# zm0612/funny_lidar_slam

Hardware: AMD Instinct MI355X
Metric: scans/sec (64-ring×1800 pts → 1e6-pt iVox map), SE(3) err vs CPU ref (higher is better)
Workload: dtype f64; 1 GPU; BASELINE configs[1]: Velodyne-64 synthetic scan (64x1800 = 115,200 pts), point-to-plane (LoamPointToPlaneIVOX semantics, YAML config_nclt.yaml) into a 1e6-pt iVox map, 1 scan per GPU per step (the same scan on every GPU); scan_points=115200, map_points=1000000, converged=True, pre_warm_matches=256

## Files before the change

### funny_lidar_slam_amd/_lib.py

```python
from __future__ import annotations

import ctypes as C
import os
import subprocess

_HERE = os.path.dirname(os.path.abspath(__file__))
LIB_PATH = os.environ.get("FLS_REG_LIB") or os.path.join(_HERE, "libfls_reg.so")
CSRC_DIR = os.path.join(_HERE, "csrc")

EXPORTED_SYMBOLS = [
    "fls_create", "fls_destroy", "fls_add_cloud_to_local_map", "fls_match", "fls_get_fitness_score",
    "fls_scan_upload", "fls_scan_upload_raw", "fls_match_resident", "fls_match_batch", "fls_map_export", "fls_map_import", "fls_map_image_bytes", "fls_map_image_export", "fls_map_image_import", "fls_get_iteration_log", "fls_get_correspondences", "fls_map_size",
    "fls_set_profiling", "fls_get_kernel_time", "fls_get_traffic_counters", "fls_get_debug_stamps", "fls_debug_fullpiv_qr6", "fls_debug_ldlt6", "fls_debug_voxel_grid", "fls_debug_voxel_grid_timed", "fls_debug_exact_sort", "fls_debug_exact_sort_marks", "fls_voxel_grid_cloud", "fls_loop_match", "fls_status_string", "fls_abi_version", "fls_abi_revision",
    "fls_device_count",
    "fls_replicas_create", "fls_replicas_refresh", "fls_replicas_match_batch", "fls_replicas_import_ms", "fls_replicas_destroy",
    "fls_features_create", "fls_features_destroy", "fls_features_project", "fls_features_extract", "fls_features_get", "fls_features_get_time",
]
HANDOFF_SYMBOLS = ["fls_preprocess_scan_device", "fls_scan_attach_preprocessed", "fls_preprocess_get_host_bytes"]
PREPROCESS_SYMBOLS = [
    "fls_preprocess_create", "fls_preprocess_destroy", "fls_preprocess_scan", "fls_preprocess_get", "fls_preprocess_get_time",
    "fls_features_project_deskew",
] + HANDOFF_SYMBOLS

FLS_OK, FLS_NOT_CONVERGED, FLS_SKIPPED = 0, 1, 2
FLS_ERR_INVALID, FLS_ERR_DEVICE, FLS_ERR_RANGE, FLS_ERR_NOMEM, FLS_ERR_STATE = -1, -2, -3, -4, -5

ICP_OPTIMIZED, P2PLANE_IVOX, INCREMENTAL_NDT, LOAM_FULL, P2PLANE_KDTREE = range(5)

# ... 172 lines not shown
                                     C.c_void_p]
        L.fls_voxel_grid_cloud.restype = C.c_int
        L.fls_voxel_grid_cloud.argtypes = [C.c_int, C.c_int, C.POINTER(C.c_float), C.c_size_t, C.c_int, C.c_float, C.POINTER(C.c_float), C.c_size_t,
                                           C.POINTER(C.c_size_t)]
        L.fls_debug_voxel_grid.restype = C.c_int
        L.fls_debug_voxel_grid.argtypes = [C.c_int, C.POINTER(C.c_float), C.c_size_t, C.c_int, C.c_float, C.POINTER(C.c_float), C.c_size_t,
                                           C.POINTER(C.c_size_t)]
        L.fls_debug_voxel_grid_timed.restype = C.c_int
        L.fls_debug_voxel_grid_timed.argtypes = [C.c_int, C.POINTER(C.c_float), C.c_size_t, C.c_int, C.c_float, C.c_int, C.POINTER(C.c_double), C.POINTER(C.c_size_t)]
        L.fls_debug_exact_sort.restype = C.c_int
        L.fls_debug_exact_sort.argtypes = [C.c_int, C.POINTER(C.c_uint32), C.POINTER(C.c_uint32), C.c_size_t, C.c_int]
        L.fls_debug_fullpiv_qr6.restype = C.c_int
        L.fls_debug_fullpiv_qr6.argtypes = [C.c_int, C.POINTER(C.c_double), C.POINTER(C.c_double), C.c_int, C.POINTER(C.c_double)]
        L.fls_debug_ldlt6.restype = C.c_int
        L.fls_debug_ldlt6.argtypes = [C.c_int, C.POINTER(C.c_double), C.POINTER(C.c_double), C.c_int, C.POINTER(C.c_double), C.POINTER(C.c_int32)]
        L.fls_get_debug_stamps.restype = C.c_int
        L.fls_get_debug_stamps.argtypes = [hp, C.POINTER(C.c_int64)]
        L.fls_features_create.restype = C.c_int
        L.fls_features_create.argtypes = [C.POINTER(FeatureParams), C.c_int, C.POINTER(hp)]
        L.fls_features_destroy.restype = None
        L.fls_features_destroy.argtypes = [hp]
        L.fls_features_project.restype = C.c_int
        L.fls_features_project.argtypes = [hp, C.c_void_p, C.c_size_t, C.POINTER(PointLayout), C.POINTER(C.c_size_t)]
        L.fls_features_extract.restype = C.c_int
        L.fls_features_extract.argtypes = [hp, C.POINTER(C.c_size_t), C.POINTER(C.c_size_t)]
        L.fls_features_get.restype = C.c_size_t
        L.fls_features_get.argtypes = [hp, C.c_int, C.c_void_p, C.c_size_t]
        L.fls_features_get_time.restype = C.c_int
        L.fls_features_get_time.argtypes = [hp, dp, dp]
        u64p = C.POINTER(C.c_uint64)
# ... 35 lines not shown
```

### funny_lidar_slam_amd/csrc/device_common.hpp

```cpp
#pragma once
#include <hip/hip_runtime.h>
#include <stdint.h>

namespace fls {

constexpr int kMaxIter = 64;
constexpr int kPartialStride = 32;
constexpr unsigned long long kEmptyKey = ~0ull;
constexpr int kKeyLimit = (1 << 20) - 2;

struct HashEntry {
    unsigned long long key;
    unsigned begin;
    unsigned count;
};
static_assert(sizeof(HashEntry) == 16, "one dwordx4 per probe");

struct DevGrid {
    const HashEntry* table;
    const float4* pts;
    unsigned mask;
    unsigned n_pts;
};

// ... 162 lines not shown
}
__host__ __device__ __forceinline__ void unpack_key(unsigned long long k, int& x, int& y, int& z) {
    x = (int)((unsigned)(k >> 42) << 11) >> 11;
    y = (int)((unsigned)((k >> 21) & 0x1FFFFFu) << 11) >> 11;
    z = (int)((unsigned)(k & 0x1FFFFFu) << 11) >> 11;
}
__host__ __device__ __forceinline__ unsigned hash_key(unsigned long long k) {
    k ^= k >> 33;
    k *= 0xff51afd7ed558ccdULL;
    k ^= k >> 33;
    k *= 0xc4ceb9fe1a85ec53ULL;
    k ^= k >> 33;
    return (unsigned)k;
}

__device__ __forceinline__ unsigned evict_merged_rank(const unsigned* __restrict__ crank, const unsigned C, const unsigned* S, const unsigned nS, const unsigned k) {
    unsigned j = 0;
    while (j < nS && j <= k && S[j] < (k - j < C ? crank[k - j] : 0xFFFFFFFFu)) ++j;
    unsigned v = 0u;
    if (j <= k && k - j < C) v = crank[k - j];
    if (j > 0u && S[j - 1] > v) v = S[j - 1];
    return v;
}

}
```

### funny_lidar_slam_amd/csrc/fls_reg.hip

```cpp
#include <chrono>
#include "matcher_p2plane_ivox.hpp"
#include "matchers_kd.hpp"
#include "matcher_ndt.hpp"
#include "features_host.hpp"
#include "preprocess_host.hpp"
#include "loop_closure.hpp"
#include "replicas.hpp"
#include <new>

using namespace fls;

namespace {

int gfx950_device_count() {
    int n = 0;
    if (hipGetDeviceCount(&n) != hipSuccess) return 0;
    int ok = 0;
    for (int d = 0; d < n; ++d) {
        hipDeviceProp_t prop;
        if (hipGetDeviceProperties(&prop, d) != hipSuccess) continue;
        if (std::strncmp(prop.gcnArchName, "gfx950", 6) == 0) ++ok;
    }
    return ok;
}
// ... 263 lines not shown
    if (launches) *launches = h->prof_launches;
    if (point_iters) *point_iters = h->prof_point_iters;
    h->prof_ms = 0.0;
    h->prof_launches = 0;
    h->prof_point_iters = 0;
    return FLS_OK;
}

fls_status fls_get_debug_stamps(fls_handle h, int64_t out[16]) {
    if (!h || !out || !h->h_state.p) return FLS_ERR_INVALID;
    (void)guarded([&]() -> fls_status { FLS_HIP(hipSetDevice(h->device)); h->refresh_log(); return FLS_OK; });
    for (int i = 0; i < 16; ++i) out[i] = h->h_state.p->dbg[i];
    return FLS_OK;
}

fls_status fls_debug_fullpiv_qr6(int device_id, const double* H, const double* g, int n, double* x) {
    if (!H || !g || !x || n < 0) return FLS_ERR_INVALID;
    if (n == 0) return FLS_OK;
    return guarded([&]() -> fls_status {
        FLS_HIP(hipSetDevice(device_id));
        DevBuf<double> dH, dg, dx;
        dH.reserve(size_t(n) * 36); dg.reserve(size_t(n) * 6); dx.reserve(size_t(n) * 6);
        FLS_HIP(hipMemcpy(dH.p, H, size_t(n) * 36 * sizeof(double), hipMemcpyHostToDevice));
        FLS_HIP(hipMemcpy(dg.p, g, size_t(n) * 6 * sizeof(double), hipMemcpyHostToDevice));
        hipLaunchKernelGGL(debug_fullpiv_qr6_kernel, dim3(unsigned(n)), dim3(64), 0, nullptr, (const double*)dH.p, (const double*)dg.p, n, dx.p);
        FLS_HIP(hipGetLastError());
        FLS_HIP(hipMemcpy(x, dx.p, size_t(n) * 6 * sizeof(double), hipMemcpyDeviceToHost));
        return FLS_OK;
    });
}
// ... 303 lines not shown
```

### funny_lidar_slam_amd/csrc/kernels_ivox_coop.hpp

```cpp
#pragma once
#include "kernels_p2plane.hpp"

namespace fls {

__device__ __forceinline__ void nearby18(const int k, int& dx, int& dy, int& dz) {
    constexpr unsigned long long DX = 0x1548889561ull, DY = 0x895429495ull, DZ = 0x282956155ull;
    dx = (int)((DX >> (2 * k)) & 3ull) - 1;
    dy = (int)((DY >> (2 * k)) & 3ull) - 1;
    dz = (int)((DZ >> (2 * k)) & 3ull) - 1;
}

template <int STEP>
__device__ __forceinline__ unsigned dpp_pair_u32(const unsigned v) {
    static_assert(STEP >= 0 && STEP <= 3, "");
    if (STEP == 0) return (unsigned)__builtin_amdgcn_update_dpp(0, (int)v, 0xB1, 0xf, 0xf, true);
    if (STEP == 1) return (unsigned)__builtin_amdgcn_update_dpp(0, (int)v, 0x4E, 0xf, 0xf, true);
    if (STEP == 2) return (unsigned)__builtin_amdgcn_update_dpp(0, (int)v, 0x141, 0xf, 0xf, true);
    return (unsigned)__builtin_amdgcn_update_dpp(0, (int)v, 0x140, 0xf, 0xf, true);
}
template <int G>
__device__ __forceinline__ unsigned long long group_min_u64(unsigned long long v) {
#define FLS_MIN_STEP(S)                                                                               \
    {                                                                                                 \
        const unsigned lo = dpp_pair_u32<S>((unsigned)(v & 0xffffffffull));                          \
// ... 64 lines not shown
#undef FLS_DMIN_STEP
    return v;
}

template <int R>
__device__ __forceinline__ unsigned slot_select(const unsigned idx, const unsigned p1, const unsigned p2, const unsigned p3, const unsigned p4,
                                                const unsigned o0, const unsigned o1, const unsigned o2, const unsigned o3, const unsigned o4) {
    unsigned sel = R == 5 ? o4 : R == 4 ? o3 : R == 3 ? o2 : R == 2 ? o1 : o0;
    if (R > 4) sel = idx < p4 ? o3 : sel;
    if (R > 3) sel = idx < p3 ? o2 : sel;
    if (R > 2) sel = idx < p2 ? o1 : sel;
    if (R > 1) sel = idx < p1 ? o0 : sel;
    return idx + sel;
}

template <int G, bool COUNT, bool DENSE, bool FIRST, bool BAL = false>
__global__ void __launch_bounds__(256)
ivox_knn_kernel(const float* __restrict__ sx, const float* __restrict__ sy, const float* __restrict__ sz, const int n,
                const GnState* __restrict__ st, const Pose16 T0, const DevGrid grid, const BrickDir bd,
                const float inv_res, float4* __restrict__ nn_pts , unsigned char* __restrict__ nn_cnt,
                unsigned char* __restrict__ flag, TrafficCounters* __restrict__ tc, const int chunk,
                unsigned* __restrict__ nn_ids ,
                const int nn_prev ,
                float* __restrict__ dev_copy ) {
    static_assert(G == 4 || G == 8, "group size");
    constexpr int QPB = 256 / G;
    constexpr int R = (19 + G - 1) / G;
    const int nb = (n + QPB - 1) / QPB;
    const int xcd = blockIdx.x & 7, seq = blockIdx.x >> 3;
    const int lb = ((seq / chunk) * 8 + xcd) * chunk + (seq % chunk);
    const int sub = threadIdx.x % G;
    const int q = lb * QPB + threadIdx.x / G;
    const bool active = lb < nb && q < n;
    const int done = FIRST ? 0 : st->done;
    double T[12];
#pragma unroll
    for (int c = 0; c < 4; ++c)
#pragma unroll
        for (int r = 0; r < 3; ++r) T[c * 3 + r] = FIRST ? T0.m[c * 4 + r] : st->T[c * 4 + r];
    const int qq = active ? q : 0;
    const float px = sx[qq], py = sy[qq], pz = sz[qq];
    if (done) return;
    if (FIRST && active && sub == 0) {
        if (dev_copy) { dev_copy[q] = px; dev_copy[(size_t)n + q] = py; dev_copy[2 * (size_t)n + q] = pz; }
        flag[q] = 0;
        if (q >= nn_prev) nn_cnt[q] = 0;
    }
    const double x = px, y = py, z = pz;
    const float ptx = (float)(((T[0] * x + T[3] * y) + T[6] * z) + T[9]);
    const float pty = (float)(((T[1] * x + T[4] * y) + T[7] * z) + T[10]);
    const float ptz = (float)(((T[2] * x + T[5] * y) + T[8] * z) + T[11]);
    const float fx = roundf(ptx * inv_res), fy = roundf(pty * inv_res), fz = roundf(ptz * inv_res);
    const bool in_range = active && fabsf(fx) < (float)kKeyLimit && fabsf(fy) < (float)kKeyLimit && fabsf(fz) < (float)kKeyLimit;
    const int kx = in_range ? (int)fx : 0, ky = in_range ? (int)fy : 0, kz = in_range ? (int)fz : 0;

    const double kNone = __hiloint2double((int)kKeyNoneHi, -1);
    double t5[5] = {kNone, kNone, kNone, kNone, kNone};
    unsigned long long c_hits = 0, c_cand = 0, c_probes = 0;
    auto probe_key = [&](const int r, bool& pv) -> unsigned long long {
        const int k = sub + G * r;
        pv = in_range && k < 19;
// ... 130 lines not shown
    }
    const double m0 = group_min_dkey<G>(t5[0]);
    if (dkey_valid(m0)) {
        int cnt = 0;
        double mine = kNone;
        unsigned sid[5] = {~0u, ~0u, ~0u, ~0u, ~0u};
#pragma unroll
        for (int j = 0; j < 5; ++j) {
            const double m = j == 0 ? m0 : group_min_dkey<G>(t5[0]);
            const bool mv = dkey_valid(m);
            cnt += mv ? 1 : 0;
            if (mv && __double_as_longlong(t5[0]) == __double_as_longlong(m)) {
                t5[0] = t5[1]; t5[1] = t5[2]; t5[2] = t5[3]; t5[3] = t5[4]; t5[4] = kNone;
            }
            if (G >= 8) { if (sub == j) mine = m; }
            else if (nn_ids) sid[j] = mv ? dkey_slot(m) : ~0u;
            else if (sub == 0 && active) {
                nn_pts[(size_t)q * 5 + j] = mv ? grid.pts[dkey_slot(m)] : make_float4(0.f, 0.f, 0.f, __int_as_float(-1));
            }
        }
        if (nn_ids) {
            if (G >= 8) { if (sub < 5 && active) nn_ids[(size_t)q * 8 + sub] = dkey_valid(mine) ? dkey_slot(mine) : ~0u; }
            else if (sub == 0 && active) {
                *reinterpret_cast<uint4*>(nn_ids + (size_t)q * 8) = make_uint4(sid[0], sid[1], sid[2], sid[3]);
                nn_ids[(size_t)q * 8 + 4] = sid[4];
            }
            if (sub == 0 && active) nn_cnt[q] = (unsigned char)cnt;
        } else {
            if (G >= 8 && sub < 5 && active)
                nn_pts[(size_t)q * 5 + sub] = dkey_valid(mine) ? grid.pts[dkey_slot(mine)] : make_float4(0.f, 0.f, 0.f, __int_as_float(-1));
            if (sub == 0 && active) nn_cnt[q] = (unsigned char)(cnt | 0x80);
        }
    }
    if (COUNT) {
        const double p = wave_sum_u((double)c_probes), hsum = wave_sum_u((double)c_hits), c = wave_sum_u((double)c_cand);
        if ((threadIdx.x & 63) == 0) {
            atomicAdd(&tc->probes, (unsigned long long)p);
            atomicAdd(&tc->hits, (unsigned long long)hsum);
            atomicAdd(&tc->cand, (unsigned long long)c);
        }
    }
}

constexpr int kFitThreads = 512;
template <bool FIRST, int NT = kFitThreads>
__global__ void __launch_bounds__(NT)
p2plane_fit_solve_kernel(const float* __restrict__ sx, const float* __restrict__ sy, const float* __restrict__ sz, const int n,
                         GnState* __restrict__ st, const Pose16 T0, const float4* __restrict__ nn_pts,
                         const unsigned char* __restrict__ nn_cnt, double* __restrict__ Jst , unsigned char* __restrict__ flag,
                         double* __restrict__ partials, unsigned* __restrict__ ticket, Mailbox* __restrict__ mb, const unsigned match_id,
                         const double plane_thres, const double rot_thr, const double pos_thr, const int shards,
                         const unsigned* __restrict__ nn_ids , const float4* __restrict__ map_pts, const unsigned n_slots) {
    const int i = blockIdx.x * NT + threadIdx.x;
    const int done = FIRST ? 0 : st->done;
    double T44[16];
#pragma unroll
    for (int k = 0; k < 16; ++k) T44[k] = FIRST ? T0.m[k] : st->T[k];
    const double last_rot = FIRST ? 0.0 : st->last_rot, last_pos = FIRST ? 0.0 : st->last_pos;
    const int it = FIRST ? 0 : st->iter;
    const int ii = i < n ? i : 0;
    const int cb = nn_cnt[ii];
    const int cnt = cb & 7;
    float4 nn[5];
    if (nn_ids) {
        const uint4 i4 = *reinterpret_cast<const uint4*>(nn_ids + (size_t)ii * 8);
        const unsigned i5 = nn_ids[(size_t)ii * 8 + 4];
        const unsigned sl[5] = {i4.x, i4.y, i4.z, i4.w, i5};
        const bool rows_form = (cb & 0x80) != 0;
#pragma unroll
        for (int j = 0; j < 5; ++j) {
            const float4* src = rows_form ? nn_pts + (size_t)ii * 5 + j : map_pts + (sl[j] < n_slots ? sl[j] : 0u);
            nn[j] = *src;
        }
    } else {
#pragma unroll
        for (int j = 0; j < 5; ++j) nn[j] = nn_pts[(size_t)ii * 5 + j];
    }
    const float px = sx[ii], py = sy[ii], pz = sz[ii];
    const unsigned char stale = FIRST ? (unsigned char)0 : flag[ii];
// ... 94 lines not shown

__global__ void __launch_bounds__(256)
ivox_apply_updates_kernel(const PtUpdDev* __restrict__ pu, const int npu, const CellUpdDev* __restrict__ cu, const int ncu,
                          float4* __restrict__ pts, uint2* __restrict__ cells) {
    const int i = blockIdx.x * 256 + threadIdx.x;
    if (i < npu) {
        const PtUpdDev u = pu[i];
        pts[u.slot] = make_float4(u.x, u.y, u.z, __int_as_float(u.id));
    }
    if (i < ncu) {
        const CellUpdDev u = cu[i];
        cells[u.idx] = make_uint2(u.begin, u.count);
    }
}

__global__ void __launch_bounds__(256)
ivox_nn_materialize_kernel(const unsigned* __restrict__ nn_ids, unsigned char* __restrict__ nn_cnt, const int n, const float4* __restrict__ map_pts,
                           const unsigned n_slots, float4* __restrict__ nn_pts) {
    const int i = blockIdx.x * 256 + threadIdx.x;
    if (i >= n) return;
    const unsigned char cb = nn_cnt[i];
    if (cb & 0x80) return;
    if (cb & 7) {
#pragma unroll
        for (int j = 0; j < 5; ++j) {
            const unsigned sl = nn_ids[(size_t)i * 8 + j];
            nn_pts[(size_t)i * 5 + j] = sl < n_slots ? map_pts[sl] : make_float4(0.f, 0.f, 0.f, __int_as_float(-1));
        }
    }
    nn_cnt[i] = (unsigned char)(cb | 0x80);
}

template <bool MATERIALIZE>
__global__ void __launch_bounds__(256)
ivox_add_decide_kernel(const float* __restrict__ sx, const float* __restrict__ sy, const float* __restrict__ sz, const int n,
                       const Pose16 Tw, float4* __restrict__ nn_pts, unsigned char* __restrict__ nn_cnt, const int nn_n,
                       const double fs , unsigned char* __restrict__ code, float4* __restrict__ pw_out,
                       const unsigned* __restrict__ nn_ids , const float4* __restrict__ map_pts, const unsigned n_slots,
                       uint2* __restrict__ lx , uint2* __restrict__ bt, unsigned* __restrict__ st_status,
                       unsigned* __restrict__ st_apply, const GnState* __restrict__ gn , const int max_it) {
    Pose16 Tl = Tw;
    if (gn != nullptr) {
        const bool go = (gn->done != 0 || gn->iter >= max_it) && gn->n_valid >= 50;
        if (!go) {
            if (blockIdx.x == 0 && threadIdx.x == 0) { *st_status = 16u; *st_apply = 0u; }
            return;
        }
#pragma unroll
        for (int q = 0; q < 16; ++q) Tl.m[q] = gn->T[q];
    }
    const int i = blockIdx.x * 256 + threadIdx.x;
    unsigned char c = 0;
    if (i < n || (MATERIALIZE && i < nn_n)) {
        const int cb = i < nn_n ? nn_cnt[i] : 0;
        const int cnt = cb & 7;
        const bool ids_form = nn_ids != nullptr && !(cb & 0x80);
        float4 nb[5];
        if (MATERIALIZE) {
#pragma unroll
            for (int k = 0; k < 5; ++k) {
                if (ids_form) {
                    const unsigned sl = nn_ids[(size_t)i * 8 + k];
                    nb[k] = (cnt && sl < n_slots) ? map_pts[sl] : make_float4(0.f, 0.f, 0.f, __int_as_float(-1));
                } else {
                    nb[k] = (i < nn_n && cnt) ? nn_pts[(size_t)i * 5 + k] : make_float4(0.f, 0.f, 0.f, __int_as_float(-1));
                }
            }
            if (i < nn_n && ids_form) {
                if (cnt) {
#pragma unroll
                    for (int k = 0; k < 5; ++k) nn_pts[(size_t)i * 5 + k] = nb[k];
                }
                nn_cnt[i] = (unsigned char)(cb | 0x80);
            }
        }
        if (i < n) {
            const double x = sx[i], y = sy[i], z = sz[i];
            const float wx = (float)(((Tl.m[0] * x + Tl.m[4] * y) + Tl.m[8] * z) + Tl.m[12]);
            const float wy = (float)(((Tl.m[1] * x + Tl.m[5] * y) + Tl.m[9] * z) + Tl.m[13]);
            const float wz = (float)(((Tl.m[2] * x + Tl.m[6] * y) + Tl.m[10] * z) + Tl.m[14]);
            pw_out[i] = make_float4(wx, wy, wz, 0.f);
            auto neighbour = [&](const int k) -> float4 {
                if (MATERIALIZE) return nb[k];
                if (!ids_form) return nn_pts[(size_t)i * 5 + k];
                const unsigned sl = nn_ids[(size_t)i * 8 + k];
                return map_pts[sl < n_slots ? sl : 0u];
            };
            c = 1;
            if (cnt > 0) {
                const double half = 0.5 * fs;
                const double c0 = (floor((double)wx / fs) + 0.5) * fs, c1 = (floor((double)wy / fs) + 0.5) * fs, c2 = (floor((double)wz / fs) + 0.5) * fs;
                const float4 n0 = neighbour(0);
                const double d0 = (double)n0.x - c0, d1 = (double)n0.y - c1, d2 = (double)n0.z - c2;
                if (fabs(d0) > half && fabs(d1) > half && fabs(d2) > half) {
                    c = 2;
                } else {
                    const double e0 = (double)wx - c0, e1 = (double)wy - c1, e2 = (double)wz - c2;
                    const double dist = (e0 * e0 + e1 * e1) + e2 * e2;
                    bool need_add = true;
                    if (cnt >= 5) {
// ... 26 lines not shown
```

### funny_lidar_slam_amd/csrc/matcher_p2plane_ivox.hpp

```cpp
#pragma once
#include "matcher_base.hpp"
#include "kernels_p2plane.hpp"
#include "kernels_knn.hpp"
#include "kernels_ivox_coop.hpp"
#include "kernels_ivox_update.hpp"
#include "ivox_image.hpp"
#include "fitness_host.hpp"
#include "device_voxelgrid.hpp"
#include <thread>
#include <chrono>
#include <hip/hip_ext.h>

namespace fls {

constexpr int kIvoxXcdChunk = 8;

struct P2PlaneIvoxMatcher final : fls_matcher {
    HostIvox ivox;
    IvoxImage image;
    bool image_dirty = true, image_built = false;
    bool rebuild_after_replay = false;
    size_t n_incremental = 0, n_full_rebuilds = 0;
    const IvoxImage* borrowed = nullptr;
    bool replica_only = false;
// ... 18 lines not shown
    DevBuf<unsigned char> d_fbit;
    PinnedBuf<char> upd_stage;
    DevBuf<unsigned char> d_code;
    DevBuf<float4> d_pw;
    std::vector<unsigned char> h_code;
    std::vector<Pt4> h_pw;
    DevBuf<unsigned> d_ticket;
    bool use_dense = true;
    bool is_first = true;
    const double filter_size_map_min = 0.5;

    DevScan scan;
    DevBuf<float4> d_nn;
    DevBuf<unsigned char> d_nn_cnt;
    DevBuf<unsigned> d_nn_ids;
    bool nn_rows_current = true;
    size_t nn_n = 0;
    int nn_prev = 0;
    DevBuf<double> d_J;
    DevBuf<unsigned char> d_flag;
    size_t number_planar_point = 0;
    double T_[16]{}, final_T[16]{};
    bool have_final = false;
    CellGridImage fitness_grid;
    bool have_fitness_grid = false;
    std::vector<Pt4> h_nn;
    std::vector<unsigned char> h_cnt, h_flag;

    ~P2PlaneIvoxMatcher() override {
        if (stream) (void)hipStreamSynchronize(stream);
// ... 185 lines not shown
        return true;
    }

    static PtI xform_d(const PtI& p, const double* T) {
        PtI r = p;
        const double x = p.x, y = p.y, z = p.z;
        r.x = float(((T[0] * x + T[4] * y) + T[8] * z) + T[12]);
        r.y = float(((T[1] * x + T[5] * y) + T[9] * z) + T[13]);
        r.z = float(((T[2] * x + T[6] * y) + T[10] * z) + T[14]);
        return r;
    }

    void ensure_nn_rows() {
        if (nn_rows_current || nn_n == 0) { nn_rows_current = true; return; }
        const IvoxImage& im = borrowed ? *borrowed : image;
        hipLaunchKernelGGL(ivox_nn_materialize_kernel, dim3(unsigned((nn_n + 255) / 256)), dim3(256), 0, stream, (const unsigned*)d_nn_ids.p, d_nn_cnt.p, int(nn_n),
                           (const float4*)im.d_pts.p, unsigned(im.d_pts.cap), d_nn.p);
        FLS_HIP(hipGetLastError());
        nn_rows_current = true;
    }
    void download_nn() {
        ensure_nn_rows();
        const size_t n = nn_n;
        h_nn.resize(n * 5);
        h_cnt.resize(n);
        if (n == 0) return;
        FLS_HIP(hipMemcpyAsync(h_nn.data(), d_nn.p, n * 5 * sizeof(float4), hipMemcpyDeviceToHost, stream));
        FLS_HIP(hipMemcpyAsync(h_cnt.data(), d_nn_cnt.p, n, hipMemcpyDeviceToHost, stream));
        FLS_HIP(hipStreamSynchronize(stream));
        for (unsigned char& c : h_cnt) c &= 7;
    }

    fls_status add_cloud(const float* c0, size_t n0, const float* c1, size_t n1, int stride) override {
        if (c1 != nullptr && n1 != 0) return FLS_ERR_INVALID;
// ... 3 lines not shown

    bool launch_decide(const size_t n, const bool speculative) {
        d_code.reserve(n);
        d_pw.reserve(n);
        Pose16 Tw;
        std::memcpy(Tw.m, T_, sizeof(Tw.m));
        const GnState* const gn = speculative ? (const GnState*)d_state.p : nullptr;
        const int max_it = int(p.max_iterations);
        const int nb = int((n + kUpdBlock - 1) / kUpdBlock);
        const bool count_here = device_map && nb <= kUpdMaxBlocks;
        if (count_here) { d_lx.reserve(n); d_bt.reserve(size_t(nb)); }
        uint2* const lx_arg = count_here ? d_lx.p : nullptr;
        uint2* const bt_arg = count_here ? d_bt.p : nullptr;
        unsigned* const st_status = count_here ? &d_upd_state.p->status : nullptr;
        unsigned* const st_apply = count_here ? &d_upd_state.p->apply : nullptr;
        if ((speculative || !nn_rows_current) && nn_n > 0) {
            const size_t m = std::max(n, nn_n);
            hipLaunchKernelGGL(ivox_add_decide_kernel<true>, dim3(unsigned((m + 255) / 256)), dim3(256), 0, stream, scan.x.p, scan.y.p, scan.z.p,
                               int(n), Tw, d_nn.p, d_nn_cnt.p, int(nn_n), filter_size_map_min,
                               d_code.p, d_pw.p, (const unsigned*)d_nn_ids.p, (const float4*)image.d_pts.p, unsigned(image.d_pts.cap), lx_arg, bt_arg, st_status, st_apply, gn, max_it);
            if (!speculative) nn_rows_current = true;
        } else {
            hipLaunchKernelGGL(ivox_add_decide_kernel<false>, dim3(unsigned((n + 255) / 256)), dim3(256), 0, stream, scan.x.p, scan.y.p, scan.z.p,
                               int(n), Tw, d_nn.p, d_nn_cnt.p, int(nn_n), filter_size_map_min,
                               d_code.p, d_pw.p, (const unsigned*)d_nn_ids.p, (const float4*)image.d_pts.p, unsigned(image.d_pts.cap), lx_arg, bt_arg,
                               st_status, st_apply, gn, max_it);
        }
        FLS_HIP(hipGetLastError());
        return count_here;
    }

    fls_status add_cloud_impl(const std::vector<PtI>& planar_cloud, const bool from_resident_scan = false, const bool pre_enqueued = false) {
        if (replica_only) return FLS_ERR_STATE;
        if (p.is_localization_mode) { device_map = false; is_first = true; ivox.clear(); image_built = false; }
        fls_status rc = FLS_OK;
        if (!(from_resident_scan && !is_first)) { ensure_nn_rows(); sync_host_from_device(); }
        if (is_first) {
            rc = ivox.add_points(planar_cloud.data(), planar_cloud.size());
            if (rc != FLS_OK) return rc;
            is_first = false;
        } else if (from_resident_scan) {
            std::vector<PtI> to_add, no_downsample;
// ... 118 lines not shown
        scan_in_staging = false;
        scan.attach_device(c, stream, false);
        return FLS_OK;
    }

    void launch_knn(const size_t n, const int first, const Pose16& T0, const DevGrid& g, const BrickDir& win, hipEvent_t e0, hipEvent_t e1) {
        constexpr int G = 4;
        const bool from_host = first && scan_in_staging;
        const float* const hx = from_host ? scan.stage_dev() : nullptr;
        const float* const src_x = from_host ? hx : (const float*)scan.x.p;
        const float* const src_y = from_host ? hx + n : (const float*)scan.y.p;
        const float* const src_z = from_host ? hx + 2 * n : (const float*)scan.z.p;
        float* const dev_copy = from_host ? scan.xyz.p : nullptr;
        const size_t nblk = (n * G + 255) / 256, gran = size_t(8) * size_t(kIvoxXcdChunk);
        const dim3 grid(unsigned((nblk + gran - 1) / gran * gran));
#define FLS_KNN_L(C, D, F)                                                                                                           \
    hipExtLaunchKernelGGL((ivox_knn_kernel<G, C, D, F, true>), grid, dim3(256), 0, stream, e0, e1, 0, src_x, src_y, src_z, int(n),      \
                          (const GnState*)d_state.p, T0, g, win, ivox.inv_resolution, d_nn.p, d_nn_cnt.p, d_flag.p, d_tc.p, kIvoxXcdChunk, \
                          d_nn_ids.p, nn_prev, dev_copy)
#define FLS_KNN(C, D) do { if (first) FLS_KNN_L(C, D, true); else FLS_KNN_L(C, D, false); } while (0)
        if (win.cells) { if (count_traffic) FLS_KNN(true, true); else FLS_KNN(false, true); }
        else { if (count_traffic) FLS_KNN(true, false); else FLS_KNN(false, false); }
#undef FLS_KNN_L
#undef FLS_KNN
    }

    fls_status match_resident(double* T, int update_map, fls_stats* out) override {
        if (replica_only && update_map) return FLS_ERR_STATE;
        const size_t n = scan.n;
        number_planar_point = n;
        stats = fls_stats{};
        stats.n_source = int(n);
        std::memcpy(T_, T, sizeof(T_));
        if (n == 0) {
            stats.iterations = 1; stats.converged = 0;
            if (out) *out = stats;
            log_n = 0; log_stale = false;
            if (h_state.p) {
                std::memcpy(h_state.p->log_T[0], T, sizeof(double) * 16);
                h_state.p->log_nv[0] = 0; h_state.p->log_res[0] = 0.0; h_state.p->iter = 1;
                log_n = 1;
            }
            return FLS_NOT_CONVERGED;
        }
        if (!borrowed) refresh_image();
        const IvoxImage& im = borrowed ? *borrowed : image;
        d_nn.reserve(n * 5, true, stream);
        d_nn_cnt.reserve(n, true, stream);
        d_nn_ids.reserve(n * 8, true, stream);
        nn_prev = int(std::min(nn_n, n));
        nn_n = n;
        d_J.reserve(7 * n);
        d_flag.reserve(n);
        const int fit_threads = n <= 65536 ? 256 : kFitThreads;
        const int nwg = int((n + size_t(fit_threads) - 1) / size_t(fit_threads));
        d_partials_b.reserve(size_t(nwg) * kPartialStride);
        const int iters = int(p.max_iterations);
        const DevGrid g = im.dev();
        const BrickDir win = use_dense ? im.bricks() : BrickDir{nullptr, 0u, nullptr, 0u};
        Pose16 T0;
        std::memcpy(T0.m, T, sizeof(T0.m));
        const bool spec = update_map && !p.is_localization_mode && !borrowed && !is_first && device_map &&
                          dev_n_alive + n < ivox.capacity && int((n + kUpdBlock - 1) / kUpdBlock) <= kUpdMaxBlocks;
        spec_pending = false;
        auto after_chunk = [&](int) {
            if (!spec) return;
            if (spec_pending) ++n_speculative_skipped;
            const bool counted = launch_decide(n, true);
            spec_pending = counted && enqueue_update_chain(n, counted);
            ++n_speculative;
        };
        const unsigned word = run_mailbox_loop(iters, n, [&](int it, int first) {
            launch_knn(n, first, T0, g, win, profiling ? ev[2 * it] : nullptr, profiling ? ev[2 * it + 1] : nullptr);
#define FLS_FIT_NT(F, NT)                                                                                                            \
    hipExtLaunchKernelGGL((p2plane_fit_solve_kernel<F, NT>), dim3(nwg), dim3(NT), 0, stream, nullptr, nullptr, 0, scan.x.p, scan.y.p, scan.z.p, int(n), \
                       d_state.p, T0, (const float4*)d_nn.p, (const unsigned char*)d_nn_cnt.p, d_J.p, d_flag.p, d_partials_b.p,     \
                       d_ticket.p, mb_dev, launch_word(), p.point_to_planar_thres, p.rotation_converge_thres, p.position_converge_thres, \
                       kTicketShards, (const unsigned*)d_nn_ids.p, (const float4*)g.pts, unsigned(im.d_pts.cap))
#define FLS_FIT(F) do { if (fit_threads == 256) FLS_FIT_NT(F, 256); else FLS_FIT_NT(F, kFitThreads); } while (0)
            if (first) FLS_FIT(true); else FLS_FIT(false);
#undef FLS_FIT_NT
#undef FLS_FIT
        }, after_chunk);
        scan_in_staging = false;
        nn_rows_current = false;
        const Mailbox& mb = *mb_host;
        const int used = int(word & 0xffu);
        std::memcpy(T, mb.T, sizeof(double) * 16);
        std::memcpy(T_, mb.T, sizeof(T_));
        std::memcpy(final_T, mb.T, sizeof(final_T));
        have_final = true;
        bool has_converge = true;
        if (mb.n_valid < 50) has_converge = false;
        stats.iterations = used;
        stats.n_valid = mb.n_valid;
// ... 175 lines not shown
    std::unique_ptr<fls_matcher> clone_for_lane() override {
        auto q = std::make_unique<P2PlaneIvoxMatcher>();
        q->kind = kind; q->p = p; q->device = device;
        if (q->init() != FLS_OK) return nullptr;
        q->borrowed = &image;
        return q;
    }
    fls_status prepare_batch() override {
        refresh_image();
        FLS_HIP(hipStreamSynchronize(stream));
        return FLS_OK;
    }
    void tune_lane(fls_matcher& l) override {
        auto& q = static_cast<P2PlaneIvoxMatcher&>(l);
        q.use_dense = use_dense;
    }

    fls_status fitness(float max_range, float* score) override {
        if (!p.is_localization_mode) { *score = std::numeric_limits<float>::max(); return FLS_OK; }
        if (!have_fitness_grid || !have_final) return FLS_ERR_STATE;
        return fitness_score_device(*this, fitness_grid, scan, final_T, max_range, score);
    }

    int correspondences(int, int32_t* ids, uint8_t* cnt, uint8_t* valid, size_t cap) override {
        download_nn();
        const size_t n = std::min(cap, nn_n);
        h_flag.resize(nn_n);
        if (nn_n) {
            FLS_HIP(hipMemcpyAsync(h_flag.data(), d_flag.p, nn_n, hipMemcpyDeviceToHost, stream));
            FLS_HIP(hipStreamSynchronize(stream));
// ... 30 lines not shown
```

### funny_lidar_slam_amd/registration.py

```python
from __future__ import annotations

import ctypes as C
from dataclasses import dataclass, field

import numpy as np

from . import _lib
from ._lib import FlsError, Params, Stats

FloatNaN = float(np.finfo(np.float32).max)

kPointToPlane_IVOX_HIP = "PointToPlane_IVOX_HIP"
kPointToPlane_KdTree_HIP = "PointToPlane_KdTree_HIP"
kLoamFull_KdTree_HIP = "LoamFull_KdTree_HIP"
kIcpOptimized_HIP = "IcpOptimized_HIP"
kIncrementalNDT_HIP = "IncrementalNDT_HIP"


@dataclass
class PointcloudCluster:
    ordered_cloud_: np.ndarray = field(default_factory=lambda: np.zeros((0, 3), np.float32))
    planar_cloud_: np.ndarray = field(default_factory=lambda: np.zeros((0, 3), np.float32))
    corner_cloud_: np.ndarray = field(default_factory=lambda: np.zeros((0, 3), np.float32))
    raw_cloud_: np.ndarray = None
# ... 181 lines not shown
    def MapImageBytes(self) -> int:
        return int(_lib.lib().fls_map_image_bytes(self._h))

    def ExportMapImage(self, ptr: int, nbytes: int, on_device: bool) -> None:
        rc = _lib.lib().fls_map_image_export(self._h, C.c_void_p(ptr), nbytes, 1 if on_device else 0)
        if rc != _lib.FLS_OK:
            raise FlsError(rc, "fls_map_image_export")

    def ImportMapImage(self, ptr: int, nbytes: int, on_device: bool) -> None:
        rc = _lib.lib().fls_map_image_import(self._h, C.c_void_p(ptr), nbytes, 1 if on_device else 0)
        if rc != _lib.FLS_OK:
            raise FlsError(rc, "fls_map_image_import")

    def map_size(self, slot: int = 0) -> int:
        return int(_lib.lib().fls_map_size(self._h, slot))

    def set_profiling(self, events: bool, counters: bool = False) -> None:
        _lib.lib().fls_set_profiling(self._h, (1 if events else 0) | (2 if counters else 0))

    def kernel_time(self):
        ms = C.c_double(); n = C.c_int64(); pi = C.c_uint64()
        _lib.lib().fls_get_kernel_time(self._h, C.byref(ms), C.byref(n), C.byref(pi))
        return ms.value, n.value, pi.value

    def traffic_counters(self):
        a = C.c_uint64(); b = C.c_uint64(); c = C.c_uint64()
        _lib.lib().fls_get_traffic_counters(self._h, C.byref(a), C.byref(b), C.byref(c))
        return a.value, b.value, c.value

    def close(self) -> None:
# ... 212 lines not shown
```

### include/fls_reg.h

```cpp
#ifndef FLS_REG_H
#define FLS_REG_H
#include <stddef.h>
#include <stdint.h>
#ifdef __cplusplus
extern "C" {
#endif

#define FLS_ABI_VERSION 1
#define FLS_ABI_REVISION 9

typedef enum fls_kind {
    FLS_ICP_OPTIMIZED = 0,
    FLS_P2PLANE_IVOX = 1,
    FLS_INCREMENTAL_NDT = 2,
    FLS_LOAM_FULL = 3,
    FLS_P2PLANE_KDTREE = 4
} fls_kind;

typedef enum fls_status {
    FLS_OK = 0,
    FLS_NOT_CONVERGED = 1,
    FLS_SKIPPED = 2,
    FLS_ERR_INVALID = -1,
    FLS_ERR_DEVICE = -2,
// ... 100 lines not shown

fls_status fls_set_profiling(fls_handle h, int enable);
fls_status fls_get_kernel_time(fls_handle h, double* ms_total, int64_t* launches, uint64_t* point_iters);
fls_status fls_get_traffic_counters(fls_handle h, uint64_t* probes, uint64_t* hit_voxels, uint64_t* cand_points);

fls_status fls_get_debug_stamps(fls_handle h, int64_t out[16]);

fls_status fls_debug_fullpiv_qr6(int device_id, const double* H, const double* g, int n, double* x);

fls_status fls_debug_ldlt6(int device_id, const double* H, const double* g, int n, double* x, int32_t* ok);

fls_status fls_debug_voxel_grid(int device_id, const float* pts, size_t n, int stride, float leaf, float* out, size_t cap, size_t* n_out);
fls_status fls_debug_voxel_grid_timed(int device_id, const float* pts, size_t n, int stride, float leaf, int reps, double* ms, size_t* n_out);
fls_status fls_debug_exact_sort(int device_id, uint32_t* key, uint32_t* val, size_t n, int on_host);
int fls_debug_exact_sort_marks(unsigned* out, int n);

const char* fls_status_string(int status);
int fls_abi_version(void);
int fls_abi_revision(void);
int fls_device_count(void);

#ifdef __cplusplus
}
#endif
#endif
```

Measured before the change: 10000 scans/s.

## Pack five 25-bit neighbour slot ids and count into one 16-byte word

Replaces the per-query neighbour handoff (8 uint ids plus a separate count byte) with a single uint4 holding five 25-bit slot indices and a 3-bit count, and uses a sentinel count for the materialized-rows form. The kNN, fit/solve, materialize and add-decide kernels read and write this packed word whenever the map slot capacity fits in 2^25. The goal is to halve the handoff traffic and drop the separate count load in the fit kernel. The cost is extra bit unpacking, a mode-switch kernel, and added code complexity around the rows/ids form transitions.

```diff
diff --git a/funny_lidar_slam_amd/_lib.py b/funny_lidar_slam_amd/_lib.py
--- a/funny_lidar_slam_amd/_lib.py
+++ b/funny_lidar_slam_amd/_lib.py
@@ -11,7 +11,7 @@
 EXPORTED_SYMBOLS = [
     "fls_create", "fls_destroy", "fls_add_cloud_to_local_map", "fls_match", "fls_get_fitness_score",
     "fls_scan_upload", "fls_scan_upload_raw", "fls_match_resident", "fls_match_batch", "fls_map_export", "fls_map_import", "fls_map_image_bytes", "fls_map_image_export", "fls_map_image_import", "fls_get_iteration_log", "fls_get_correspondences", "fls_map_size",
-    "fls_set_profiling", "fls_get_kernel_time", "fls_get_traffic_counters", "fls_get_debug_stamps", "fls_debug_fullpiv_qr6", "fls_debug_ldlt6", "fls_debug_voxel_grid", "fls_debug_voxel_grid_timed", "fls_debug_exact_sort", "fls_debug_exact_sort_marks", "fls_voxel_grid_cloud", "fls_loop_match", "fls_status_string", "fls_abi_version", "fls_abi_revision",
+    "fls_set_profiling", "fls_get_kernel_time", "fls_get_traffic_counters", "fls_get_debug_stamps", "fls_debug_fullpiv_qr6", "fls_debug_ldlt6", "fls_debug_voxel_grid", "fls_debug_voxel_grid_timed", "fls_debug_exact_sort", "fls_debug_exact_sort_marks", "fls_debug_set_nn_pack_limit", "fls_voxel_grid_cloud", "fls_loop_match", "fls_status_string", "fls_abi_version", "fls_abi_revision",
     "fls_device_count",
     "fls_replicas_create", "fls_replicas_refresh", "fls_replicas_match_batch", "fls_replicas_import_ms", "fls_replicas_destroy",
     "fls_features_create", "fls_features_destroy", "fls_features_project", "fls_features_extract", "fls_features_get", "fls_features_get_time",
@@ -214,6 +214,9 @@
         L.fls_debug_fullpiv_qr6.argtypes = [C.c_int, C.POINTER(C.c_double), C.POINTER(C.c_double), C.c_int, C.POINTER(C.c_double)]
         L.fls_debug_ldlt6.restype = C.c_int
         L.fls_debug_ldlt6.argtypes = [C.c_int, C.POINTER(C.c_double), C.POINTER(C.c_double), C.c_int, C.POINTER(C.c_double), C.POINTER(C.c_int32)]
+        if hasattr(L, "fls_debug_set_nn_pack_limit"):
+            L.fls_debug_set_nn_pack_limit.restype = C.c_int
+            L.fls_debug_set_nn_pack_limit.argtypes = [hp, C.c_int]
         L.fls_get_debug_stamps.restype = C.c_int
         L.fls_get_debug_stamps.argtypes = [hp, C.POINTER(C.c_int64)]
         L.fls_features_create.restype = C.c_int
diff --git a/funny_lidar_slam_amd/csrc/device_common.hpp b/funny_lidar_slam_amd/csrc/device_common.hpp
--- a/funny_lidar_slam_amd/csrc/device_common.hpp
+++ b/funny_lidar_slam_amd/csrc/device_common.hpp
@@ -200,6 +200,31 @@
     return (unsigned)k;
 }
 
+constexpr int kNnSlotBits = 25;
+constexpr int kNnPackMaxLog2 = kNnSlotBits;
+constexpr unsigned kNnSlotMask = (1u << kNnSlotBits) - 1u;
+constexpr unsigned kNnRowsMark = 7u;
+__host__ __device__ __forceinline__ uint4 nn_pack(const unsigned s0, const unsigned s1, const unsigned s2, const unsigned s3, const unsigned s4,
+                                                  const unsigned cnt) {
+    uint4 w;
+    w.x = s0 | (s1 << 25);
+    w.y = (s1 >> 7) | (s2 << 18);
+    w.z = (s2 >> 14) | (s3 << 11);
+    w.w = (s3 >> 21) | (s4 << 4) | (cnt << 29);
+    return w;
+}
+__host__ __device__ __forceinline__ void nn_unpack(const uint4 w, unsigned (&s)[5], unsigned& cnt) {
+    s[0] = w.x & kNnSlotMask;
+    s[1] = ((w.x >> 25) | (w.y << 7)) & kNnSlotMask;
+    s[2] = ((w.y >> 18) | (w.z << 14)) & kNnSlotMask;
+    s[3] = ((w.z >> 11) | (w.w << 21)) & kNnSlotMask;
+    s[4] = (w.w >> 4) & kNnSlotMask;
+    cnt = w.w >> 29;
+}
+__host__ __device__ __forceinline__ uint4 nn_pack_rows(const unsigned cnt) { return nn_pack(cnt, 0u, 0u, 0u, 0u, kNnRowsMark); }
+__host__ __device__ __forceinline__ bool nn_word_rows(const uint4 w) { return (w.w >> 29) == kNnRowsMark; }
+__host__ __device__ __forceinline__ unsigned nn_word_count(const uint4 w) { return nn_word_rows(w) ? (w.x & 7u) : (w.w >> 29); }
+
 __device__ __forceinline__ unsigned evict_merged_rank(const unsigned* __restrict__ crank, const unsigned C, const unsigned* S, const unsigned nS, const unsigned k) {
     unsigned j = 0;
     while (j < nS && j <= k && S[j] < (k - j < C ? crank[k - j] : 0xFFFFFFFFu)) ++j;
diff --git a/funny_lidar_slam_amd/csrc/fls_reg.hip b/funny_lidar_slam_amd/csrc/fls_reg.hip
--- a/funny_lidar_slam_amd/csrc/fls_reg.hip
+++ b/funny_lidar_slam_amd/csrc/fls_reg.hip
@@ -301,6 +301,12 @@
     return FLS_OK;
 }
 
+fls_status fls_debug_set_nn_pack_limit(fls_handle h, int log2_slots) {
+    if (!h || h->kind != FLS_P2PLANE_IVOX || log2_slots < 0 || log2_slots > kNnPackMaxLog2) return FLS_ERR_INVALID;
+    static_cast<P2PlaneIvoxMatcher*>(h)->nn_pack_log2 = log2_slots;
+    return FLS_OK;
+}
+
 fls_status fls_debug_fullpiv_qr6(int device_id, const double* H, const double* g, int n, double* x) {
     if (!H || !g || !x || n < 0) return FLS_ERR_INVALID;
     if (n == 0) return FLS_OK;
diff --git a/funny_lidar_slam_amd/csrc/kernels_ivox_coop.hpp b/funny_lidar_slam_amd/csrc/kernels_ivox_coop.hpp
--- a/funny_lidar_slam_amd/csrc/kernels_ivox_coop.hpp
+++ b/funny_lidar_slam_amd/csrc/kernels_ivox_coop.hpp
@@ -102,7 +102,7 @@
     return idx + sel;
 }
 
-template <int G, bool COUNT, bool DENSE, bool FIRST, bool BAL = false>
+template <int G, bool COUNT, bool DENSE, bool FIRST, bool BAL = false, bool PACK = false>
 __global__ void __launch_bounds__(256)
 ivox_knn_kernel(const float* __restrict__ sx, const float* __restrict__ sy, const float* __restrict__ sz, const int n,
                 const GnState* __restrict__ st, const Pose16 T0, const DevGrid grid, const BrickDir bd,
@@ -112,6 +112,7 @@
                 const int nn_prev ,
                 float* __restrict__ dev_copy ) {
     static_assert(G == 4 || G == 8, "group size");
+    static_assert(!(PACK && G >= 8), "the packed hand-off is built for 4 lanes per query; G == 8 keeps the wide form");
     constexpr int QPB = 256 / G;
     constexpr int R = (19 + G - 1) / G;
     const int nb = (n + QPB - 1) / QPB;
@@ -132,7 +133,10 @@
     if (FIRST && active && sub == 0) {
         if (dev_copy) { dev_copy[q] = px; dev_copy[(size_t)n + q] = py; dev_copy[2 * (size_t)n + q] = pz; }
         flag[q] = 0;
-        if (q >= nn_prev) nn_cnt[q] = 0;
+        if (q >= nn_prev) {
+            if (PACK) reinterpret_cast<uint4*>(nn_ids)[q] = make_uint4(0u, 0u, 0u, 0u);
+            else nn_cnt[q] = 0;
+        }
     }
     const double x = px, y = py, z = pz;
     const float ptx = (float)(((T[0] * x + T[3] * y) + T[6] * z) + T[9]);
@@ -293,12 +297,15 @@
                 t5[0] = t5[1]; t5[1] = t5[2]; t5[2] = t5[3]; t5[3] = t5[4]; t5[4] = kNone;
             }
             if (G >= 8) { if (sub == j) mine = m; }
+            else if (PACK) sid[j] = mv ? dkey_slot(m) : 0u;
             else if (nn_ids) sid[j] = mv ? dkey_slot(m) : ~0u;
             else if (sub == 0 && active) {
                 nn_pts[(size_t)q * 5 + j] = mv ? grid.pts[dkey_slot(m)] : make_float4(0.f, 0.f, 0.f, __int_as_float(-1));
             }
         }
-        if (nn_ids) {
+        if (PACK) {
+            if (sub == 0 && active) reinterpret_cast<uint4*>(nn_ids)[q] = nn_pack(sid[0], sid[1], sid[2], sid[3], sid[4], (unsigned)cnt);
+        } else if (nn_ids) {
             if (G >= 8) { if (sub < 5 && active) nn_ids[(size_t)q * 8 + sub] = dkey_valid(mine) ? dkey_slot(mine) : ~0u; }
             else if (sub == 0 && active) {
                 *reinterpret_cast<uint4*>(nn_ids + (size_t)q * 8) = make_uint4(sid[0], sid[1], sid[2], sid[3]);
@@ -322,14 +329,15 @@
 }
 
 constexpr int kFitThreads = 512;
-template <bool FIRST, int NT = kFitThreads>
+template <bool FIRST, int NT = kFitThreads, bool PACK = false>
 __global__ void __launch_bounds__(NT)
 p2plane_fit_solve_kernel(const float* __restrict__ sx, const float* __restrict__ sy, const float* __restrict__ sz, const int n,
                          GnState* __restrict__ st, const Pose16 T0, const float4* __restrict__ nn_pts,
                          const unsigned char* __restrict__ nn_cnt, double* __restrict__ Jst , unsigned char* __restrict__ flag,
                          double* __restrict__ partials, unsigned* __restrict__ ticket, Mailbox* __restrict__ mb, const unsigned match_id,
                          const double plane_thres, const double rot_thr, const double pos_thr, const int shards,
-                         const unsigned* __restrict__ nn_ids , const float4* __restrict__ map_pts, const unsigned n_slots) {
+                         const unsigned* __restrict__ nn_ids , const float4* __restrict__ map_pts,
+                         const unsigned n_slots) {
     const int i = blockIdx.x * NT + threadIdx.x;
     const int done = FIRST ? 0 : st->done;
     double T44[16];
@@ -338,10 +346,27 @@
     const double last_rot = FIRST ? 0.0 : st->last_rot, last_pos = FIRST ? 0.0 : st->last_pos;
     const int it = FIRST ? 0 : st->iter;
     const int ii = i < n ? i : 0;
-    const int cb = nn_cnt[ii];
-    const int cnt = cb & 7;
+    const int cb = PACK ? 0 : nn_cnt[ii];
+    int cnt = cb & 7;
     float4 nn[5];
-    if (nn_ids) {
+    if (PACK) {
+        const uint4 w = reinterpret_cast<const uint4*>(nn_ids)[ii];
+        const unsigned cf = w.w >> 29;
+        const bool rows_form = cf == kNnRowsMark;
+        cnt = (int)(rows_form ? (w.x & 7u) : cf);
+        const float4* const rows = nn_pts + (size_t)ii * 5;
+#define FLS_NN_GATHER(J, SLOT)                                                          \
+        {                                                                               \
+            const unsigned sl = (SLOT) & kNnSlotMask;                                   \
+            nn[J] = *(rows_form ? rows + J : map_pts + (sl < n_slots ? sl : 0u));       \
+        }
+        FLS_NN_GATHER(0, w.x)
+        FLS_NN_GATHER(1, (w.x >> 25) | (w.y << 7))
+        FLS_NN_GATHER(2, (w.y >> 18) | (w.z << 14))
+        FLS_NN_GATHER(3, (w.z >> 11) | (w.w << 21))
+        FLS_NN_GATHER(4, w.w >> 4)
+#undef FLS_NN_GATHER
+    } else if (nn_ids) {
         const uint4 i4 = *reinterpret_cast<const uint4*>(nn_ids + (size_t)ii * 8);
         const unsigned i5 = nn_ids[(size_t)ii * 8 + 4];
         const unsigned sl[5] = {i4.x, i4.y, i4.z, i4.w, i5};
@@ -466,11 +491,26 @@
     }
 }
 
+template <bool PACK>
 __global__ void __launch_bounds__(256)
-ivox_nn_materialize_kernel(const unsigned* __restrict__ nn_ids, unsigned char* __restrict__ nn_cnt, const int n, const float4* __restrict__ map_pts,
+ivox_nn_materialize_kernel(unsigned* __restrict__ nn_ids, unsigned char* __restrict__ nn_cnt, const int n, const float4* __restrict__ map_pts,
                            const unsigned n_slots, float4* __restrict__ nn_pts) {
     const int i = blockIdx.x * 256 + threadIdx.x;
     if (i >= n) return;
+    if (PACK) {
+        const uint4 w = reinterpret_cast<const uint4*>(nn_ids)[i];
+        unsigned s[5], cf;
+        nn_unpack(w, s, cf);
+        if (cf == kNnRowsMark) return;
+        if (cf) {
+#pragma unroll
+            for (int j = 0; j < 5; ++j)
+                nn_pts[(size_t)i * 5 + j] = ((unsigned)j < cf && s[j] < n_slots) ? map_pts[s[j]] : make_float4(0.f, 0.f, 0.f, __int_as_float(-1));
+        }
+        reinterpret_cast<uint4*>(nn_ids)[i] = nn_pack_rows(cf);
+        nn_cnt[i] = (unsigned char)(cf | 0x80);
+        return;
+    }
     const unsigned char cb = nn_cnt[i];
     if (cb & 0x80) return;
     if (cb & 7) {
@@ -483,12 +523,18 @@
     nn_cnt[i] = (unsigned char)(cb | 0x80);
 }
 
-template <bool MATERIALIZE>
+__global__ void __launch_bounds__(256)
+ivox_nn_mark_rows_kernel(const unsigned char* __restrict__ nn_cnt, uint4* __restrict__ nn_words, const int n) {
+    const int i = blockIdx.x * 256 + threadIdx.x;
+    if (i < n) nn_words[i] = nn_pack_rows(nn_cnt[i] & 7u);
+}
+
+template <bool MATERIALIZE, bool PACK = false>
 __global__ void __launch_bounds__(256)
 ivox_add_decide_kernel(const float* __restrict__ sx, const float* __restrict__ sy, const float* __restrict__ sz, const int n,
                        const Pose16 Tw, float4* __restrict__ nn_pts, unsigned char* __restrict__ nn_cnt, const int nn_n,
                        const double fs , unsigned char* __restrict__ code, float4* __restrict__ pw_out,
-                       const unsigned* __restrict__ nn_ids , const float4* __restrict__ map_pts, const unsigned n_slots,
+                       unsigned* __restrict__ nn_ids , const float4* __restrict__ map_pts, const unsigned n_slots,
                        uint2* __restrict__ lx , uint2* __restrict__ bt, unsigned* __restrict__ st_status,
                        unsigned* __restrict__ st_apply, const GnState* __restrict__ gn , const int max_it) {
     Pose16 Tl = Tw;
@@ -504,15 +550,30 @@
     const int i = blockIdx.x * 256 + threadIdx.x;
     unsigned char c = 0;
     if (i < n || (MATERIALIZE && i < nn_n)) {
-        const int cb = i < nn_n ? nn_cnt[i] : 0;
-        const int cnt = cb & 7;
-        const bool ids_form = nn_ids != nullptr && !(cb & 0x80);
+        int cb, cnt;
+        bool ids_form;
+        unsigned sl5[5] = {~0u, ~0u, ~0u, ~0u, ~0u};
+        if (PACK) {
+            const uint4 w = i < nn_n ? reinterpret_cast<const uint4*>(nn_ids)[i] : make_uint4(0u, 0u, 0u, 0u);
+            unsigned s[5], cf;
+            nn_unpack(w, s, cf);
+            ids_form = cf != kNnRowsMark;
+            cnt = (int)(ids_form ? cf : (s[0] & 7u));
+            cb = cnt;
+#pragma unroll
+            for (int k = 0; k < 5; ++k) sl5[k] = (ids_form && k < cnt) ? s[k] : ~0u;
+        } else {
+            cb = i < nn_n ? nn_cnt[i] : 0;
+            cnt = cb & 7;
+            ids_form = nn_ids != nullptr && !(cb & 0x80);
+        }
+        auto slot_at = [&](const int k) -> unsigned { return PACK ? sl5[k] : nn_ids[(size_t)i * 8 + k]; };
         float4 nb[5];
         if (MATERIALIZE) {
 #pragma unroll
             for (int k = 0; k < 5; ++k) {
                 if (ids_form) {
-                    const unsigned sl = nn_ids[(size_t)i * 8 + k];
+                    const unsigned sl = slot_at(k);
                     nb[k] = (cnt && sl < n_slots) ? map_pts[sl] : make_float4(0.f, 0.f, 0.f, __int_as_float(-1));
                 } else {
                     nb[k] = (i < nn_n && cnt) ? nn_pts[(size_t)i * 5 + k] : make_float4(0.f, 0.f, 0.f, __int_as_float(-1));
@@ -524,6 +585,7 @@
                     for (int k = 0; k < 5; ++k) nn_pts[(size_t)i * 5 + k] = nb[k];
                 }
                 nn_cnt[i] = (unsigned char)(cb | 0x80);
+                if (PACK) reinterpret_cast<uint4*>(nn_ids)[i] = nn_pack_rows((unsigned)cnt);
             }
         }
         if (i < n) {
@@ -535,7 +597,7 @@
             auto neighbour = [&](const int k) -> float4 {
                 if (MATERIALIZE) return nb[k];
                 if (!ids_form) return nn_pts[(size_t)i * 5 + k];
-                const unsigned sl = nn_ids[(size_t)i * 8 + k];
+                const unsigned sl = slot_at(k);
                 return map_pts[sl < n_slots ? sl : 0u];
             };
             c = 1;
diff --git a/funny_lidar_slam_amd/csrc/matcher_p2plane_ivox.hpp b/funny_lidar_slam_amd/csrc/matcher_p2plane_ivox.hpp
--- a/funny_lidar_slam_amd/csrc/matcher_p2plane_ivox.hpp
+++ b/funny_lidar_slam_amd/csrc/matcher_p2plane_ivox.hpp
@@ -56,6 +56,8 @@
     DevBuf<float4> d_nn;
     DevBuf<unsigned char> d_nn_cnt;
     DevBuf<unsigned> d_nn_ids;
+    bool nn_packed = false;
+    int nn_pack_log2 = kNnPackMaxLog2;
     bool nn_rows_current = true;
     size_t nn_n = 0;
     int nn_prev = 0;
@@ -271,10 +273,27 @@
     void ensure_nn_rows() {
         if (nn_rows_current || nn_n == 0) { nn_rows_current = true; return; }
         const IvoxImage& im = borrowed ? *borrowed : image;
-        hipLaunchKernelGGL(ivox_nn_materialize_kernel, dim3(unsigned((nn_n + 255) / 256)), dim3(256), 0, stream, (const unsigned*)d_nn_ids.p, d_nn_cnt.p, int(nn_n),
-                           (const float4*)im.d_pts.p, unsigned(im.d_pts.cap), d_nn.p);
+        const dim3 grid(unsigned((nn_n + 255) / 256));
+        if (nn_packed)
+            hipLaunchKernelGGL(ivox_nn_materialize_kernel<true>, grid, dim3(256), 0, stream, d_nn_ids.p, d_nn_cnt.p, int(nn_n), (const float4*)im.d_pts.p,
+                               unsigned(im.d_pts.cap), d_nn.p);
+        else
+            hipLaunchKernelGGL(ivox_nn_materialize_kernel<false>, grid, dim3(256), 0, stream, d_nn_ids.p, d_nn_cnt.p, int(nn_n), (const float4*)im.d_pts.p,
+                               unsigned(im.d_pts.cap), d_nn.p);
         FLS_HIP(hipGetLastError());
         nn_rows_current = true;
+    }
+    void select_nn_form(const IvoxImage& im) {
+        const bool pack = im.d_pts.cap <= (size_t(1) << nn_pack_log2);
+        if (pack == nn_packed) return;
+        ensure_nn_rows();
+        if (pack && nn_n) {
+            d_nn_ids.reserve(nn_n * 4, false, stream);
+            hipLaunchKernelGGL(ivox_nn_mark_rows_kernel, dim3(unsigned((nn_n + 255) / 256)), dim3(256), 0, stream, (const unsigned char*)d_nn_cnt.p,
+                               reinterpret_cast<uint4*>(d_nn_ids.p), int(nn_n));
+            FLS_HIP(hipGetLastError());
+        }
+        nn_packed = pack;
     }
     void download_nn() {
         ensure_nn_rows();
@@ -308,18 +327,18 @@
         uint2* const bt_arg = count_here ? d_bt.p : nullptr;
         unsigned* const st_status = count_here ? &d_upd_state.p->status : nullptr;
         unsigned* const st_apply = count_here ? &d_upd_state.p->apply : nullptr;
+#define FLS_DECIDE(M, P, CNT)                                                                                                                \
+    hipLaunchKernelGGL((ivox_add_decide_kernel<M, P>), dim3(unsigned(((CNT) + 255) / 256)), dim3(256), 0, stream, scan.x.p, scan.y.p, scan.z.p, int(n), \
+                       Tw, d_nn.p, d_nn_cnt.p, int(nn_n), filter_size_map_min, d_code.p, d_pw.p, d_nn_ids.p, (const float4*)image.d_pts.p,        \
+                       unsigned(image.d_pts.cap), lx_arg, bt_arg, st_status, st_apply, gn, max_it)
         if ((speculative || !nn_rows_current) && nn_n > 0) {
             const size_t m = std::max(n, nn_n);
-            hipLaunchKernelGGL(ivox_add_decide_kernel<true>, dim3(unsigned((m + 255) / 256)), dim3(256), 0, stream, scan.x.p, scan.y.p, scan.z.p,
-                               int(n), Tw, d_nn.p, d_nn_cnt.p, int(nn_n), filter_size_map_min,
-                               d_code.p, d_pw.p, (const unsigned*)d_nn_ids.p, (const float4*)image.d_pts.p, unsigned(image.d_pts.cap), lx_arg, bt_arg, st_status, st_apply, gn, max_it);
+            if (nn_packed) FLS_DECIDE(true, true, m); else FLS_DECIDE(true, false, m);
             if (!speculative) nn_rows_current = true;
         } else {
-            hipLaunchKernelGGL(ivox_add_decide_kernel<false>, dim3(unsigned((n + 255) / 256)), dim3(256), 0, stream, scan.x.p, scan.y.p, scan.z.p,
-                               int(n), Tw, d_nn.p, d_nn_cnt.p, int(nn_n), filter_size_map_min,
-                               d_code.p, d_pw.p, (const unsigned*)d_nn_ids.p, (const float4*)image.d_pts.p, unsigned(image.d_pts.cap), lx_arg, bt_arg,
-                               st_status, st_apply, gn, max_it);
-        }
+            if (nn_packed) FLS_DECIDE(false, true, n); else FLS_DECIDE(false, false, n);
+        }
+#undef FLS_DECIDE
         FLS_HIP(hipGetLastError());
         return count_here;
     }
@@ -468,14 +487,16 @@
         float* const dev_copy = from_host ? scan.xyz.p : nullptr;
         const size_t nblk = (n * G + 255) / 256, gran = size_t(8) * size_t(kIvoxXcdChunk);
         const dim3 grid(unsigned((nblk + gran - 1) / gran * gran));
-#define FLS_KNN_L(C, D, F)                                                                                                           \
-    hipExtLaunchKernelGGL((ivox_knn_kernel<G, C, D, F, true>), grid, dim3(256), 0, stream, e0, e1, 0, src_x, src_y, src_z, int(n),      \
+#define FLS_KNN_L(C, D, F, P)                                                                                                         \
+    hipExtLaunchKernelGGL((ivox_knn_kernel<G, C, D, F, true, P>), grid, dim3(256), 0, stream, e0, e1, 0, src_x, src_y, src_z, int(n),      \
                           (const GnState*)d_state.p, T0, g, win, ivox.inv_resolution, d_nn.p, d_nn_cnt.p, d_flag.p, d_tc.p, kIvoxXcdChunk, \
                           d_nn_ids.p, nn_prev, dev_copy)
-#define FLS_KNN(C, D) do { if (first) FLS_KNN_L(C, D, true); else FLS_KNN_L(C, D, false); } while (0)
+#define FLS_KNN_F(C, D, F) do { if (nn_packed) FLS_KNN_L(C, D, F, true); else FLS_KNN_L(C, D, F, false); } while (0)
+#define FLS_KNN(C, D) do { if (first) FLS_KNN_F(C, D, true); else FLS_KNN_F(C, D, false); } while (0)
         if (win.cells) { if (count_traffic) FLS_KNN(true, true); else FLS_KNN(false, true); }
         else { if (count_traffic) FLS_KNN(true, false); else FLS_KNN(false, false); }
 #undef FLS_KNN_L
+#undef FLS_KNN_F
 #undef FLS_KNN
     }
 
@@ -501,7 +522,8 @@
         const IvoxImage& im = borrowed ? *borrowed : image;
         d_nn.reserve(n * 5, true, stream);
         d_nn_cnt.reserve(n, true, stream);
-        d_nn_ids.reserve(n * 8, true, stream);
+        select_nn_form(im);
+        d_nn_ids.reserve(n * (nn_packed ? 4 : 8), true, stream);
         nn_prev = int(std::min(nn_n, n));
         nn_n = n;
         d_J.reserve(7 * n);
@@ -526,13 +548,15 @@
         };
         const unsigned word = run_mailbox_loop(iters, n, [&](int it, int first) {
             launch_knn(n, first, T0, g, win, profiling ? ev[2 * it] : nullptr, profiling ? ev[2 * it + 1] : nullptr);
-#define FLS_FIT_NT(F, NT)                                                                                                            \
-    hipExtLaunchKernelGGL((p2plane_fit_solve_kernel<F, NT>), dim3(nwg), dim3(NT), 0, stream, nullptr, nullptr, 0, scan.x.p, scan.y.p, scan.z.p, int(n), \
+#define FLS_FIT_NT_P(F, NT, P)                                                                                                       \
+    hipExtLaunchKernelGGL((p2plane_fit_solve_kernel<F, NT, P>), dim3(nwg), dim3(NT), 0, stream, nullptr, nullptr, 0, scan.x.p, scan.y.p, scan.z.p, int(n), \
                        d_state.p, T0, (const float4*)d_nn.p, (const unsigned char*)d_nn_cnt.p, d_J.p, d_flag.p, d_partials_b.p,     \
                        d_ticket.p, mb_dev, launch_word(), p.point_to_planar_thres, p.rotation_converge_thres, p.position_converge_thres, \
                        kTicketShards, (const unsigned*)d_nn_ids.p, (const float4*)g.pts, unsigned(im.d_pts.cap))
+#define FLS_FIT_NT(F, NT) do { if (nn_packed) FLS_FIT_NT_P(F, NT, true); else FLS_FIT_NT_P(F, NT, false); } while (0)
 #define FLS_FIT(F) do { if (fit_threads == 256) FLS_FIT_NT(F, 256); else FLS_FIT_NT(F, kFitThreads); } while (0)
             if (first) FLS_FIT(true); else FLS_FIT(false);
+#undef FLS_FIT_NT_P
 #undef FLS_FIT_NT
 #undef FLS_FIT
         }, after_chunk);
@@ -738,6 +762,7 @@
     void tune_lane(fls_matcher& l) override {
         auto& q = static_cast<P2PlaneIvoxMatcher&>(l);
         q.use_dense = use_dense;
+        q.nn_pack_log2 = nn_pack_log2;
     }
 
     fls_status fitness(float max_range, float* score) override {
diff --git a/funny_lidar_slam_amd/registration.py b/funny_lidar_slam_amd/registration.py
--- a/funny_lidar_slam_amd/registration.py
+++ b/funny_lidar_slam_amd/registration.py
@@ -219,6 +219,11 @@
 
     def map_size(self, slot: int = 0) -> int:
         return int(_lib.lib().fls_map_size(self._h, slot))
+
+    def debug_set_nn_pack_limit(self, log2_slots: int) -> None:
+        rc = _lib.lib().fls_debug_set_nn_pack_limit(self._h, int(log2_slots))
+        if rc != _lib.FLS_OK:
+            raise _lib.FlsError(rc, "fls_debug_set_nn_pack_limit")
 
     def set_profiling(self, events: bool, counters: bool = False) -> None:
         _lib.lib().fls_set_profiling(self._h, (1 if events else 0) | (2 if counters else 0))
diff --git a/include/fls_reg.h b/include/fls_reg.h
--- a/include/fls_reg.h
+++ b/include/fls_reg.h
@@ -138,6 +138,7 @@
 fls_status fls_debug_voxel_grid_timed(int device_id, const float* pts, size_t n, int stride, float leaf, int reps, double* ms, size_t* n_out);
 fls_status fls_debug_exact_sort(int device_id, uint32_t* key, uint32_t* val, size_t n, int on_host);
 int fls_debug_exact_sort_marks(unsigned* out, int n);
+fls_status fls_debug_set_nn_pack_limit(fls_handle h, int log2_slots);
 
 const char* fls_status_string(int status);
 int fls_abi_version(void);
```

Result: slower. 9563 scans/s (-4.4%).
